# raulmur/ORB_SLAM

Measured on AMD Instinct MI355X. Metric: frames/s ORB extract+match @640x480, 1000 kp, higher is better.
Workload: dtype u8; 1 GPU; vga: 640x480 grayscale stream, 8 levels, nFeatures 1000, S-blocks frames, extract + Hamming top-2 match vs previous frame (BASELINE.json configs[1] + the frame-to-frame match of the metric); resident_frames_per_gpu=2048, lanes=4, parity_checked_frames=0, parity_mismatches=0, library_build_id=8ff709f66bece802, lane_placement=2

## Files before the change

### orb_slam_amd/csrc/k_describe_od.hip

```cpp
#include <algorithm>
#include <type_traits>

#include "orbx_device.h"

namespace orbx {

constexpr int OD_KPW = 4;
constexpr int OD_PITCH = 48, OD_ROWS = 43;
constexpr int OD_WIN_BYTES = OD_PITCH * OD_ROWS;
constexpr int OD_CHUNKS = OD_ROWS * 3;
constexpr int OD_WAVES = DESC_WAVES;
constexpr int OD_TAIL = 512;

typedef int v4i __attribute__((ext_vector_type(4)));
typedef float f2v __attribute__((ext_vector_type(2)));
__device__ __forceinline__ int float_bits(float v) { return __builtin_bit_cast(int, v); }
__host__ __device__ constexpr int od_col0(int ct) { return ct == 0 ? 0 : ct == 1 ? 16 : 24; }
__host__ __device__ constexpr int od_row0(int rt) { return rt == 0 ? 0 : rt == 1 ? 16 : 21; }
typedef const void __attribute__((address_space(1))) * gptr_t;
typedef void __attribute__((address_space(3))) * lptr_t;

constexpr int od_tap(int t) { return t >= 0 && t <= 6 ? (int)((0x12223137312212ull >> (8 * t)) & 255ull) : 0; }
constexpr uint32_t od_taps4(int t0) { return (uint32_t)od_tap(t0) | (uint32_t)od_tap(t0 + 1) << 8 | (uint32_t)od_tap(t0 + 2) << 16 | (uint32_t)od_tap(t0 + 3) << 24; }
struct OdTables {
    uint32_t mask[256];
    float pat[256][4];
    uint32_t trow[3][64][4];
    uint32_t tcol[3][64][4];
};
constexpr uint32_t c_pattern_host[256] = {
#include "orb_pattern_packed.inc"
};
constexpr OdTables make_od_tables() {
    OdTables T{};
    for (int t = 0; t < 256; t++) {
        const int r = t >> 3, c = t & 7;
        const int v = r - HALF_PATCH, av = v < 0 ? -v : v;
        const int um = r < 31 ? (int)((UMAX_NIBBLES >> (4 * (av & 15))) & 15ull) : -1;
        uint32_t mask = 0;
        for (int kk = 0; kk < 4; kk++) {
            const int u = 4 * c + kk - HALF_PATCH;
            if ((u < 0 ? -u : u) <= um) mask |= 0xFFu << (8 * kk);
        }
        T.mask[t] = mask;
        const uint32_t pk = c_pattern_host[t];
        for (int e = 0; e < 4; e++) T.pat[t][e] = (float)(int)(int8_t)(uint8_t)(pk >> (8 * e));
    }
    for (int c = 0; c < 3; c++)
        for (int l = 0; l < 64; l++)
            for (int v = 0; v < 4; v++) {
                const int n = l & 15, g = l >> 4;
                T.trow[c][l][v] = od_taps4(16 * g + 4 * v - (od_col0(c) + n) - 1);
                T.tcol[c][l][v] = od_taps4(16 * v + 4 * g - (od_row0(c) + n));
            }
    return T;
}
static __device__ __constant__ OdTables c_od = make_od_tables();

template <bool FMA, bool GATHER>
__device__ __forceinline__ void k_describe_od_body(const Batch& b) {
    __shared__ __attribute__((aligned(16))) float s_pat[256 * 4];
    __shared__ __attribute__((aligned(16))) uint32_t s_mask[256];
    __shared__ __attribute__((aligned(16))) uint8_t s_win[OD_WAVES * OD_KPW * OD_WIN_BYTES + OD_TAIL];
    const DevGeom& g = b.g;
    int frame, wgi;
    if (!frame_item(b, blockIdx.x, (g.nquads + OD_WAVES - 1) / OD_WAVES, frame, wgi)) return;
    const int tid = threadIdx.x, lane = tid & 63;
    const int grp = lane >> 4, li = lane & 15;
    const float4 pat_first = *reinterpret_cast<const float4*>(c_od.pat[tid & 255]);
    const uint32_t mask_first = c_od.mask[tid & 255];
    const int32_t* counts = b.level_count + frame * MAX_LEVELS;
    const int quad = wgi * OD_WAVES + wave_id();
    const bool live = quad < g.nquads;
    const int level = __builtin_amdgcn_readfirstlane(find_level(g.quad_bases, live ? quad : 0));
    const LevelGeom& LG = g.lv[level];
    struct { int w, h, stride, plane_off, sel_base, quad_base, wvec; float scale, kp_size; } L = {
        __builtin_amdgcn_readfirstlane(LG.w), __builtin_amdgcn_readfirstlane(LG.h), __builtin_amdgcn_readfirstlane(LG.stride),
        __builtin_amdgcn_readfirstlane(LG.plane_off), __builtin_amdgcn_readfirstlane(LG.sel_base), __builtin_amdgcn_readfirstlane(LG.quad_base),
        __builtin_amdgcn_readfirstlane(LG.blur_wvec),
        __builtin_bit_cast(float, __builtin_amdgcn_readfirstlane(__builtin_bit_cast(int, LG.scale))),
        __builtin_bit_cast(float, __builtin_amdgcn_readfirstlane(__builtin_bit_cast(int, LG.kp_size)))};
    const int k0 = (quad - L.quad_base) * OD_KPW;
    Cand kp;
    typedef int v8i_s __attribute__((ext_vector_type(8)));
    v8i_s s_cnt0, s_cnt1;
    int st0;
    {
        const int sel_cap = __builtin_amdgcn_readfirstlane(LG.sel_cap);
        const int ks = __builtin_amdgcn_readfirstlane(max(min(k0, sel_cap - OD_KPW), 0));
        const Cand* kp4 = b.sel + ((long long)frame * g.frame_sel + L.sel_base + ks);
        const int32_t* stp = b.status + frame;
        static_assert(MAX_LEVELS >= 16, "the per-level counts are fetched as two s_load_dwordx8");
        v8i_s kq;
        int sst;
        asm volatile("s_load_dwordx8 %0, %4, 0x0\n\ts_load_dwordx8 %1, %5, 0x0\n\ts_load_dwordx8 %2, %5, 0x20\n\ts_load_dword %3, %6, 0x0\n\ts_waitcnt lgkmcnt(0)"
                     : "=&s"(kq), "=&s"(s_cnt0), "=&s"(s_cnt1), "=&s"(sst) : "s"(kp4), "s"(counts), "s"(stp) : "memory");
        st0 = sst;
        const int e = min(max(k0 + grp, 0), sel_cap - 1) - ks;
        kp.pos = (uint32_t)(e == 0 ? kq[0] : e == 1 ? kq[2] : e == 2 ? kq[4] : kq[6]);
        kp.resp = __builtin_bit_cast(float, e == 0 ? kq[1] : e == 1 ? kq[3] : e == 2 ? kq[5] : kq[7]);
    }
    static_assert(OD_WAVES * 64 == 256, "one table entry per thread");
    reinterpret_cast<float4*>(s_pat)[tid] = pat_first;
    s_mask[tid] = mask_first;
    int out_base = 0, total = 0, cnt = 0;
    for (int l = 0; l < g.nlevels; l++) {
        int c = 0;
#pragma unroll
        for (int i = 0; i < 8; i++) { if (l == i) c = s_cnt0[i]; if (l == 8 + i) c = s_cnt1[i]; }
        if (l < level) out_base += c;
        if (l == level) cnt = c;
        total += c;
    }
    const bool work = live && k0 < cnt && total <= b.cap && __builtin_amdgcn_readfirstlane(st0) == ORBX_OK;
    const bool valid = work && k0 + grp < cnt;
    const int k = valid ? k0 + grp : (work ? k0 : 0);
    if (!valid) {
        kp.pos = (uint32_t)__builtin_amdgcn_readlane((int)kp.pos, 0);
        kp.resp = __builtin_bit_cast(float, __builtin_amdgcn_readlane(__builtin_bit_cast(int, kp.resp), 0));
    }
    if (quad == 0 && lane == 0) {
        int st = st0, tot = total;
        if (tot > b.cap) { st = ORBX_ERR_CAPACITY; tot = 0; }
        b.out_n[frame] = st == ORBX_OK ? tot : 0;
        if (b.out_status) b.out_status[frame] = st;
    }
    if (!work) return;
    const int x = kp.pos & 0xFFFF, y = kp.pos >> 16;
    const uint8_t* plain;
    unsigned pstride;
    int wlim;
    if (level == 0) {
        if constexpr (GATHER) {
            long long s0;
            plain = level0_src(b, frame, s0);
            pstride = (unsigned)s0;
        } else { pstride = (unsigned)b.img_row_stride; plain = b.img + (long long)frame * b.img_frame_stride; }
        wlim = (int)min((long long)pstride, (long long)((L.w + 15) & ~15));
    } else { pstride = (unsigned)L.stride; plain = b.pyr + (long long)frame * g.frame_plane_bytes + L.plane_off; wlim = L.stride; }
    uint8_t* const win0 = s_win + wave_id() * OD_KPW * OD_WIN_BYTES;

    int erow[3], ecol[3];
    unsigned eoff[3];
#pragma unroll
    for (int n = 0; n < 3; n++) {
        const int e = 64 * n + lane;
        erow[n] = (e * 171) >> 9;
        ecol[n] = 16 * (e - 3 * erow[n]);
        eoff[n] = __umul24((unsigned)erow[n], pstride) + (unsigned)ecol[n];
    }
    uint32_t fixmask = 0;
#pragma unroll
    for (int q = 0; q < OD_KPW; q++) {
        if (q > 0 && k0 + q >= cnt) continue;
        const unsigned posq = (unsigned)__builtin_amdgcn_readlane((int)kp.pos, 16 * q);
        const int xq = posq & 0xFFFF, yq = posq >> 16;
        const int xs = (xq - 22) & ~3;
        if (xs < 0 || xs + 48 > wlim || xq + 21 >= L.w) fixmask |= 1u << q;
        if (xq < 18 || xq + 18 >= L.w || yq < 18 || yq + 21 >= L.h) fixmask |= 16u << q;
        if (xs >= 0 && xs + 48 <= wlim && yq >= 21 && yq + 21 < L.h) {
            const uint8_t* srcq = plain + (__umul24((unsigned)(yq - 21), pstride) + (unsigned)xs);
#pragma unroll
            for (int n = 0; n < 3; n++)
                if (n < 2 || lane < OD_CHUNKS - 128)
                    __builtin_amdgcn_global_load_lds((gptr_t)(srcq + eoff[n]), (lptr_t)(win0 + q * OD_WIN_BYTES + 1024 * n), 16, 0, 0);
            continue;
        }
#pragma unroll
        for (int n = 0; n < 3; n++) {
            if (n == 2 && lane >= OD_CHUNKS - 128) continue;
            int Y = yq - 21 + erow[n];
            Y = Y < 0 ? -Y : Y;
            Y = Y >= L.h ? 2 * L.h - 2 - Y : Y;
            Y = min(max(Y, 0), L.h - 1);
            const int X = min(max(xs + ecol[n], 0), wlim - 16);
            __builtin_amdgcn_global_load_lds((gptr_t)(plain + (__umul24((unsigned)Y, pstride) + (unsigned)X)), (lptr_t)(win0 + q * OD_WIN_BYTES + 1024 * n), 16, 0, 0);
        }
    }
    fixmask = (uint32_t)__builtin_amdgcn_readfirstlane((int)fixmask);
    asm volatile("s_waitcnt lgkmcnt(0)\n\ts_barrier" ::: "memory");

    const int n16 = li, g4 = grp;
    v4i Trow[3], Tcol[3];
#pragma unroll
    for (int c = 0; c < 3; c++) {
        Trow[c] = *reinterpret_cast<const v4i*>(c_od.trow[c][lane]);
        Tcol[c] = *reinterpret_cast<const v4i*>(c_od.tcol[c][lane]);
    }
    asm volatile("s_waitcnt vmcnt(0)" ::: "memory");
    wave_lds_fence();

    if (fixmask & 15u) {
#pragma unroll 1
        for (int q = 0; q < OD_KPW; q++) {
            if (!((fixmask >> q) & 1u)) continue;
            const unsigned posq = (unsigned)__builtin_amdgcn_readlane((int)kp.pos, 16 * q);
            const int xq = posq & 0xFFFF;
            const int xs = (xq - 22) & ~3;
            uint8_t* W = win0 + q * OD_WIN_BYTES;
#pragma unroll 1
            for (int j = 0; j < 3; j += 2) {
                const int X0 = xs + 16 * j, Xc = min(max(X0, 0), wlim - 16);
                if (X0 >= 0 && X0 + 16 <= wlim && X0 + 15 < L.w) continue;
                uint32_t nv[3];
#pragma unroll
                for (int it = 0; it < 3; it++) {
                    const int item = 64 * it + lane;
                    const int r = item >> 2, d = item & 3;
                    uint32_t v = 0;
                    if (item < 4 * OD_ROWS) {
#pragma unroll
                        for (int bb = 0; bb < 4; bb++) {
                            const int X = X0 + 4 * d + bb;
                            int Xr = X < 0 ? -X : (X >= L.w ? 2 * L.w - 2 - X : X);
                            Xr = min(max(Xr, 0), L.w - 1);
                            const int src = (Xr >= Xc && Xr < Xc + 16) ? 16 * j + (Xr - Xc) : min(max(Xr - xs, 0), OD_PITCH - 1);
                            v |= (uint32_t)W[r * OD_PITCH + src] << (8 * bb);
                        }
                    }
                    nv[it] = v;
                }
                wave_lds_fence();
#pragma unroll
                for (int it = 0; it < 3; it++) {
                    const int item = 64 * it + lane;
                    if (item < 4 * OD_ROWS) *reinterpret_cast<uint32_t*>(W + (item >> 2) * OD_PITCH + 16 * j + 4 * (item & 3)) = nv[it];
                }
                wave_lds_fence();
            }
        }
    }

    const int xs_own = (x - 22) & ~3, cx = x - xs_own;
    const uint8_t* Wown = win0 + grp * OD_WIN_BYTES;
    int m10, m01;
    {
        const int rsub = li >> 1, hf = li & 1;
        const int boff = cx - HALF_PATCH + 16 * hf;
        const int sh = boff & 3;
        const uint32_t* rowp = reinterpret_cast<const uint32_t*>(Wown + (6 + rsub) * OD_PITCH + (boff & ~3));
        uint32_t uw[4];
#pragma unroll
        for (int d = 0; d < 4; d++) uw[d] = (uint32_t)(16 * hf + 4 * d) * 0x01010101u + 0x03020100u;
        uint32_t a_su = 0, a_si = 0, a_r = 0;
#pragma unroll
        for (int n = 0; n < 4; n++) {
            const uint32_t* p = rowp + (8 * n) * (OD_PITCH / 4);
            uint32_t dw[5];
#pragma unroll
            for (int d = 0; d < 5; d++) dw[d] = p[d];
            const uint4 mk = *reinterpret_cast<const uint4*>(s_mask + (8 * (8 * n + rsub) + 4 * hf));
            const uint32_t mm[4] = {mk.x, mk.y, mk.z, mk.w};
            uint32_t srow = 0;
#pragma unroll
            for (int d = 0; d < 4; d++) {
                const uint32_t Im = __builtin_amdgcn_alignbyte(dw[d + 1], dw[d], (uint32_t)sh) & mm[d];
                srow = __builtin_amdgcn_udot4(Im, 0x01010101u, srow, false);
                a_su = __builtin_amdgcn_udot4(Im, uw[d], a_su, false);
            }
            a_si += srow;
            a_r = __umul24(srow, (uint32_t)(8 * n)) + a_r;
        }
        const int p10 = (int)a_su - HALF_PATCH * (int)a_si;
        const int p01 = (rsub - HALF_PATCH) * (int)a_si + (int)a_r;
        m10 = row16_sum(p10); m01 = row16_sum(p01);
    }
    const float angle = fast_atan2_deg((float)m01, (float)m10);
    wave_lds_fence();

    const unsigned a_off = (unsigned)(n16 * OD_PITCH + 16 * g4);
    const unsigned o_off = (unsigned)((n16 + 3) * OD_PITCH + 4 + 4 * g4);
    auto blur_window = [&](auto EDGE, uint8_t* W, int xs, int yq) {
        constexpr bool edge = decltype(EDGE)::value;
        v4i A[3];
        {
            const unsigned ra = (unsigned)(uintptr_t)(lptr_t)(W + a_off);
            asm volatile("ds_read_b128 %0, %3\n\tds_read_b128 %1, %3 offset:768\n\tds_read_b128 %2, %3 offset:1536\n\ts_waitcnt lgkmcnt(0)"
                         : "=&v"(A[0]), "=&v"(A[1]), "=&v"(A[2]) : "v"(ra) : "memory");
        }
#pragma unroll
        for (int t = 0; t < 3; t++) {
            A[t].x = (int)((uint32_t)A[t].x ^ 0x80808080u); A[t].y = (int)((uint32_t)A[t].y ^ 0x80808080u);
            A[t].z = (int)((uint32_t)A[t].z ^ 0x80808080u); A[t].w = (int)((uint32_t)A[t].w ^ 0x80808080u);
        }
#pragma unroll
        for (int ct = 0; ct < 3; ct++) {
            const v4i c128 = {128, 128, 128, 128};
            v4i z[3];
#pragma unroll
            for (int t = 0; t < 3; t++) z[t] = __builtin_amdgcn_mfma_i32_16x16x64_i8(A[t], Trow[ct], c128, 0, 0, 0);
            int h4[4] = {0, 0, 0, 0}, l4[4] = {0, 0, 0, 0};
#pragma unroll
            for (int t = 0; t < 3; t++) {
                const uint32_t p01 = __builtin_amdgcn_perm((uint32_t)z[t][1], (uint32_t)z[t][0], 0x05010400u);
                const uint32_t p23 = __builtin_amdgcn_perm((uint32_t)z[t][3], (uint32_t)z[t][2], 0x05010400u);
                l4[t] = (int)(__builtin_amdgcn_perm(p23, p01, 0x05040100u) ^ 0x80808080u);
                h4[t] = (int)__builtin_amdgcn_perm(p23, p01, 0x07060302u);
            }
            const v4i HI = {h4[0], h4[1], h4[2], h4[3]}, LO = {l4[0], l4[1], l4[2], l4[3]};
            const int X0 = xs + 4 + od_col0(ct) + 4 * g4;
            const uint32_t tw = X0 < L.wvec ? 1u : 0u;
            const uint32_t cadd = (uint32_t)(257 * 32896 + 0x7FFF) + (tw ^ 1u);
            uint32_t keepc = 0;
            if (edge) {
#pragma unroll
                for (int bb = 0; bb < 4; bb++) keepc |= ((unsigned)(X0 + bb) < (unsigned)L.w ? 0u : 0xFFu) << (8 * bb);
            }
#pragma unroll
            for (int rt = 0; rt < 3; rt++) {
                const v4i zero = {0, 0, 0, 0};
                v4i acc = __builtin_amdgcn_mfma_i32_16x16x64_i8(HI, Tcol[rt], zero, 0, 0, 0);
#pragma unroll
                for (int i = 0; i < 4; i++) acc[i] = (int)(((uint32_t)acc[i] << 8) + cadd);
                acc = __builtin_amdgcn_mfma_i32_16x16x64_i8(LO, Tcol[rt], acc, 0, 0, 0);
                uint32_t qv[4];
#pragma unroll
                for (int i = 0; i < 4; i++) {
                    const uint32_t t = (uint32_t)acc[i];
                    qv[i] = t + ((t >> 16) & tw);
                }
                const us2v lo2 = __builtin_elementwise_min(as_us2v(__builtin_amdgcn_perm(qv[1], qv[0], 0x07060302u)), as_us2v(0x00FF00FFu));
                const us2v hi2 = __builtin_elementwise_min(as_us2v(__builtin_amdgcn_perm(qv[3], qv[2], 0x07060302u)), as_us2v(0x00FF00FFu));
                uint32_t o = __builtin_amdgcn_perm(__builtin_bit_cast(uint32_t, hi2), __builtin_bit_cast(uint32_t, lo2), 0x06040200u);
                uint32_t* dst = reinterpret_cast<uint32_t*>(W + o_off + (od_row0(rt) * OD_PITCH + od_col0(ct)));
                if (edge) {
                    const int Y = yq - 18 + od_row0(rt) + n16;
                    const uint32_t keep = (unsigned)Y < (unsigned)L.h ? keepc : 0xFFFFFFFFu;
                    o = (o & ~keep) | (*dst & keep);
                }
                *dst = o;
            }
        }
    };
#pragma unroll 1
    for (int q = 0; q < OD_KPW; q++) {
        if (q > 0 && k0 + q >= cnt) continue;
        const unsigned posq = (unsigned)__builtin_amdgcn_readlane((int)kp.pos, 16 * q);
        const int xq = posq & 0xFFFF, yq = posq >> 16;
        const int xs = (xq - 22) & ~3;
        uint8_t* W = win0 + q * OD_WIN_BYTES;
        if ((fixmask >> (4 + q)) & 1u) blur_window(std::true_type{}, W, xs, yq);
        else blur_window(std::false_type{}, W, xs, yq);
    }
    wave_lds_fence();

    const float factorPI = (float)(3.14159265358979323846 / 180.f);
    float sn, cs;
    sincosf_orb(angle * factorPI, &sn, &cs);
    const float4* pat = reinterpret_cast<const float4*>(s_pat) + li;
    uint32_t mybits = 0;
    {
        const uint8_t* ctr = Wown + 21 * OD_PITCH + cx;
        const f2v SC = {sn, cs};
        auto rotate = [&](f2v pt) -> f2v {
            f2v m1, r;
            asm("v_pk_mul_f32 %0, %1, %2 op_sel:[1,1] op_sel_hi:[1,0]" : "=v"(m1) : "v"(pt), "v"(SC));
            if (FMA) asm("v_pk_fma_f32 %0, %1, %2, %3 op_sel:[0,0,0] op_sel_hi:[0,1,1] neg_hi:[0,0,1]" : "=v"(r) : "v"(pt), "v"(SC), "v"(m1));
            else {
                f2v m0;
                asm("v_pk_mul_f32 %0, %1, %2 op_sel:[0,0] op_sel_hi:[0,1]" : "=v"(m0) : "v"(pt), "v"(SC));
                asm("v_pk_add_f32 %0, %1, %2 neg_hi:[0,1]" : "=v"(r) : "v"(m0), "v"(m1));
            }
            return r;
        };
        f2v MAGIC = {12582912.0f, 12582912.0f};
        asm("" : "+v"(MAGIC));
        const uint32_t ctr_a = (uint32_t)(uintptr_t)(lptr_t)ctr - (uint32_t)(OD_PITCH * 0x400000 + 0x4B400000);
        typedef const uint8_t __attribute__((address_space(3))) * lbyte_t;
#pragma unroll
        for (int j = 15; j >= 0; j--) {
            const float4 P = pat[16 * j];
            f2v r0 = rotate((f2v){P.x, P.y}), r1 = rotate((f2v){P.z, P.w});
            r0 = r0 + MAGIC;
            r1 = r1 + MAGIC;
            const float r0y = r0.x, r0x = r0.y, r1y = r1.x, r1x = r1.y;
            const uint32_t o0 = (uint32_t)(__mul24(float_bits(r0y), OD_PITCH) + float_bits(r0x));
            const uint32_t o1 = (uint32_t)(__mul24(float_bits(r1y), OD_PITCH) + float_bits(r1x));
            const uint32_t v0 = *(lbyte_t)(uintptr_t)(ctr_a + o0), v1 = *(lbyte_t)(uintptr_t)(ctr_a + o1);
            asm("v_cmp_lt_u32_e32 vcc, %1, %2\n\tv_addc_co_u32_e32 %0, vcc, %0, %0, vcc" : "+v"(mybits) : "v"(v0), "v"(v1) : "vcc");
        }
    }
    uint32_t half = mybits;
    auto stage = [&](auto S) {
        constexpr int s = decltype(S)::value;
        constexpr uint32_t M0 = s == 8 ? 0x00FFu : s == 4 ? 0x0F0Fu : s == 2 ? 0x3333u : 0x5555u;
        const bool hi = (li & s) != 0;
        const uint32_t yv = (uint32_t)__builtin_amdgcn_ds_swizzle((int)half, (s << 10) | 0x1F);
        const uint32_t ysh = hi ? (yv >> s) : (yv << s);
        const uint32_t mk = hi ? (~M0 & 0xFFFFu) : M0;
        half = (half & mk) | (ysh & ~mk & 0xFFFFu);
    };
    stage(std::integral_constant<int, 8>{}); stage(std::integral_constant<int, 4>{});
    stage(std::integral_constant<int, 2>{}); stage(std::integral_constant<int, 1>{});
    if (!valid) return;
    const int out_idx = out_base + k;
    reinterpret_cast<uint16_t*>(b.out_desc + ((long long)frame * b.cap + out_idx) * 32)[li] = (uint16_t)half;
    if (li == 0) {
        orbx_keypoint o;
        o.x = (float)x; o.y = (float)y;
        if (level != 0) { o.x = o.x * L.scale; o.y = o.y * L.scale; }
        o.size = L.kp_size;
        o.angle = angle;
        o.response = kp.resp;
        o.octave = level;
        o.class_id = -1;
        b.out_kps[(long long)frame * b.cap + out_idx] = o;
    }
}
template <bool FMA>
__global__ __launch_bounds__(OD_WAVES * 64) void k_describe_od(Batch b) { k_describe_od_body<FMA, false>(b); }
template <bool FMA>
__global__ __launch_bounds__(OD_WAVES * 64) void k_describe_od_gather(Batch b) { k_describe_od_body<FMA, true>(b); }

bool describe_od_supported(const Batch& b, const HostGeom& hg) {
    const DevGeom& g = hg.g;
    for (int l = 0; l < g.nlevels; l++)
        if (g.lv[l].w < 64 || g.lv[l].h < 44) return false;
    const long long wlim0 = std::min<long long>(level0_min_stride(b), (g.lv[0].w + 15) & ~15);
    return wlim0 >= 64 && wlim0 >= g.lv[0].w;
}

int launch_describe_od(const Batch& b, const HostGeom& hg, hipStream_t stream) {
    const DevGeom& g = hg.g;
    const dim3 grid(frame_item_blocks(b, (g.nquads + OD_WAVES - 1) / OD_WAVES)), block(OD_WAVES * 64);
    if (g.fp_contract) hipLaunchKernelGGL(b.img_tab ? k_describe_od_gather<true> : k_describe_od<true>, grid, block, 0, stream, b);
    else hipLaunchKernelGGL(b.img_tab ? k_describe_od_gather<false> : k_describe_od<false>, grid, block, 0, stream, b);
    return hipGetLastError() == hipSuccess ? ORBX_OK : ORBX_ERR_DEVICE;
}

}
```

Measured before the change: 431,400 frames/s.

## Pair keypoint windows in MFMA blur to pack partial edge tiles together

Restructures the separable Gaussian blur of the four descriptor windows per wave so that windows are processed in pairs. The third, partially used column and row tiles of two windows, and a shared corner tile for all four, are packed into a single MFMA, using new zero-padded tap tables. This is meant to cut the wasted MFMA work on overlapping 16-wide edge tiles. It also switches byte packing to SDWA v_min_u16 and adds a waves_per_eu(4) occupancy hint. The price is more complex index bookkeeping, edge-case handling when paired windows disagree on bounds, and added register pressure.

```diff
diff --git a/orb_slam_amd/csrc/k_describe_od.hip b/orb_slam_amd/csrc/k_describe_od.hip
--- a/orb_slam_amd/csrc/k_describe_od.hip
+++ b/orb_slam_amd/csrc/k_describe_od.hip
@@ -15,8 +15,6 @@
 typedef int v4i __attribute__((ext_vector_type(4)));
 typedef float f2v __attribute__((ext_vector_type(2)));
 __device__ __forceinline__ int float_bits(float v) { return __builtin_bit_cast(int, v); }
-__host__ __device__ constexpr int od_col0(int ct) { return ct == 0 ? 0 : ct == 1 ? 16 : 24; }
-__host__ __device__ constexpr int od_row0(int rt) { return rt == 0 ? 0 : rt == 1 ? 16 : 21; }
 typedef const void __attribute__((address_space(1))) * gptr_t;
 typedef void __attribute__((address_space(3))) * lptr_t;
 
@@ -50,8 +48,13 @@
         for (int l = 0; l < 64; l++)
             for (int v = 0; v < 4; v++) {
                 const int n = l & 15, g = l >> 4;
-                T.trow[c][l][v] = od_taps4(16 * g + 4 * v - (od_col0(c) + n) - 1);
-                T.tcol[c][l][v] = od_taps4(16 * v + 4 * g - (od_row0(c) + n));
+                if (c < 2) {
+                    T.trow[c][l][v] = od_taps4(16 * g + 4 * v - (16 * c + n) - 1);
+                    T.tcol[c][l][v] = od_taps4(16 * v + 4 * g - (16 * c + n));
+                } else {
+                    T.trow[c][l][v] = g == 2 && n < 8 ? od_taps4(4 * v - n - 1) : g == 3 && n >= 8 ? od_taps4(4 * v - (n - 8) - 1) : 0u;
+                    T.tcol[c][l][v] = v == 2 && n < 5 ? od_taps4(4 * g - n) : v == 3 && n >= 8 && n < 13 ? od_taps4(4 * g - (n - 8)) : 0u;
+                }
             }
     return T;
 }
@@ -269,78 +272,128 @@
     wave_lds_fence();
 
     const unsigned a_off = (unsigned)(n16 * OD_PITCH + 16 * g4);
-    const unsigned o_off = (unsigned)((n16 + 3) * OD_PITCH + 4 + 4 * g4);
-    auto blur_window = [&](auto EDGE, uint8_t* W, int xs, int yq) {
-        constexpr bool edge = decltype(EDGE)::value;
-        v4i A[3];
+    const unsigned a_offp = g4 == 3 ? (unsigned)(OD_WIN_BYTES + n16 * OD_PITCH + 32) : a_off;
+    const unsigned o_own = (unsigned)((n16 + 3) * OD_PITCH + 4 + 4 * g4);
+    const unsigned o_prow = (unsigned)((n16 >= 8 ? OD_WIN_BYTES : 0) + ((n16 & 7) + 35) * OD_PITCH + 4 + 4 * g4);
+    const unsigned o_pcol = (unsigned)((g4 >= 2 ? OD_WIN_BYTES : 0) + (n16 + 3) * OD_PITCH + 36 + 4 * (g4 & 1));
+    const unsigned o_corner = (unsigned)((n16 < 8 ? 2 : 0) * OD_WIN_BYTES + (g4 >= 2 ? OD_WIN_BYTES : 0) + ((n16 & 7) + 35) * OD_PITCH + 36 + 4 * (g4 & 1));
+    int xsw[OD_KPW], yqw[OD_KPW];
+    uint32_t tww[OD_KPW];
+    bool genw[OD_KPW];
+#pragma unroll
+    for (int q = 0; q < OD_KPW; q++) {
+        const unsigned posq = (unsigned)__builtin_amdgcn_readlane((int)kp.pos, 16 * q);
+        xsw[q] = ((int)(posq & 0xFFFF) - 22) & ~3;
+        yqw[q] = (int)(posq >> 16);
+        const bool lo = xsw[q] + 4 < L.wvec, hi = xsw[q] + 40 < L.wvec;
+        const bool liveq = q == 0 || k0 + q < cnt;
+        tww[q] = liveq ? (lo ? 1u : 0u) : tww[q > 0 ? q - 1 : 0];
+        genw[q] = liveq && (((fixmask >> (4 + q)) & 1u) || lo != hi);
+    }
+    constexpr uint32_t CADD = 257 * 32896 + 0x7FFF;
+    const v4i c128 = {128, 128, 128, 128}, zero = {0, 0, 0, 0};
+    auto row_pass = [&](const v4i (&A)[3], const v4i& T, v4i& HI, v4i& LO) {
+        v4i z[3];
+#pragma unroll
+        for (int t = 0; t < 3; t++) z[t] = __builtin_amdgcn_mfma_i32_16x16x64_i8(A[t], T, c128, 0, 0, 0);
+#pragma unroll
+        for (int t = 0; t < 3; t++) {
+            const uint32_t p01 = __builtin_amdgcn_perm((uint32_t)z[t][1], (uint32_t)z[t][0], 0x05010400u);
+            const uint32_t p23 = __builtin_amdgcn_perm((uint32_t)z[t][3], (uint32_t)z[t][2], 0x05010400u);
+            LO[t] = (int)(__builtin_amdgcn_perm(p23, p01, 0x05040100u) ^ 0x80808080u);
+            HI[t] = (int)__builtin_amdgcn_perm(p23, p01, 0x07060302u);
+        }
+    };
+    const uint32_t c255 = 255;
+    auto epilogue = [&](auto GEN, const v4i& HI, const v4i& LO, const v4i& T, uint8_t* dst, int xs_l, int yq_l, int cb, int ro, uint32_t twu) {
+        constexpr bool gen = decltype(GEN)::value;
+        uint32_t tw = twu, keep = 0;
+        if (gen) {
+            const int X0 = xs_l + 4 + cb;
+            tw = X0 < L.wvec ? 1u : 0u;
+            uint32_t keepc = 0;
+#pragma unroll
+            for (int bb = 0; bb < 4; bb++) keepc |= ((unsigned)(X0 + bb) < (unsigned)L.w ? 0u : 0xFFu) << (8 * bb);
+            keep = (unsigned)(yq_l - 18 + ro) < (unsigned)L.h ? keepc : 0xFFFFFFFFu;
+        }
+        const uint32_t cadd = CADD + (tw ^ 1u);
+        v4i acc = __builtin_amdgcn_mfma_i32_16x16x64_i8(HI, T, zero, 0, 0, 0);
+#pragma unroll
+        for (int i = 0; i < 4; i++) acc[i] = (int)(((uint32_t)acc[i] << 8) + cadd);
+        acc = __builtin_amdgcn_mfma_i32_16x16x64_i8(LO, T, acc, 0, 0, 0);
+        uint32_t q[4];
+#pragma unroll
+        for (int i = 0; i < 4; i++) {
+            const uint32_t t = (uint32_t)acc[i];
+            q[i] = t + ((t >> 16) & tw);
+        }
+        uint32_t o;
+        asm("v_min_u16_sdwa %0, %1, %2 dst_sel:BYTE_0 dst_unused:UNUSED_PAD src0_sel:WORD_1 src1_sel:DWORD" : "=v"(o) : "v"(q[0]), "v"(c255));
+        asm("v_min_u16_sdwa %0, %1, %2 dst_sel:BYTE_1 dst_unused:UNUSED_PRESERVE src0_sel:WORD_1 src1_sel:DWORD" : "+v"(o) : "v"(q[1]), "v"(c255));
+        asm("v_min_u16_sdwa %0, %1, %2 dst_sel:BYTE_2 dst_unused:UNUSED_PRESERVE src0_sel:WORD_1 src1_sel:DWORD" : "+v"(o) : "v"(q[2]), "v"(c255));
+        asm("v_min_u16_sdwa %0, %1, %2 dst_sel:BYTE_3 dst_unused:UNUSED_PRESERVE src0_sel:WORD_1 src1_sel:DWORD" : "+v"(o) : "v"(q[3]), "v"(c255));
+        uint32_t* d = reinterpret_cast<uint32_t*>(dst);
+        if (gen) o = (o & ~keep) | (*d & keep);
+        *d = o;
+    };
+    int hc[2] = {0, 0}, lc[2] = {0, 0};
+    auto blur_pair = [&](auto GEN, int p, int xs0, int yq0, int xs1, int yq1, uint32_t twu) {
+        uint8_t* W = win0 + 2 * p * OD_WIN_BYTES;
+        v4i A0[3], A1[3];
         {
-            const unsigned ra = (unsigned)(uintptr_t)(lptr_t)(W + a_off);
-            asm volatile("ds_read_b128 %0, %3\n\tds_read_b128 %1, %3 offset:768\n\tds_read_b128 %2, %3 offset:1536\n\ts_waitcnt lgkmcnt(0)"
-                         : "=&v"(A[0]), "=&v"(A[1]), "=&v"(A[2]) : "v"(ra) : "memory");
-        }
-#pragma unroll
-        for (int t = 0; t < 3; t++) {
-            A[t].x = (int)((uint32_t)A[t].x ^ 0x80808080u); A[t].y = (int)((uint32_t)A[t].y ^ 0x80808080u);
-            A[t].z = (int)((uint32_t)A[t].z ^ 0x80808080u); A[t].w = (int)((uint32_t)A[t].w ^ 0x80808080u);
-        }
-#pragma unroll
-        for (int ct = 0; ct < 3; ct++) {
-            const v4i c128 = {128, 128, 128, 128};
-            v4i z[3];
-#pragma unroll
-            for (int t = 0; t < 3; t++) z[t] = __builtin_amdgcn_mfma_i32_16x16x64_i8(A[t], Trow[ct], c128, 0, 0, 0);
-            int h4[4] = {0, 0, 0, 0}, l4[4] = {0, 0, 0, 0};
-#pragma unroll
-            for (int t = 0; t < 3; t++) {
-                const uint32_t p01 = __builtin_amdgcn_perm((uint32_t)z[t][1], (uint32_t)z[t][0], 0x05010400u);
-                const uint32_t p23 = __builtin_amdgcn_perm((uint32_t)z[t][3], (uint32_t)z[t][2], 0x05010400u);
-                l4[t] = (int)(__builtin_amdgcn_perm(p23, p01, 0x05040100u) ^ 0x80808080u);
-                h4[t] = (int)__builtin_amdgcn_perm(p23, p01, 0x07060302u);
+            const unsigned r0 = (unsigned)(uintptr_t)(lptr_t)(W + a_offp), r1 = (unsigned)(uintptr_t)(lptr_t)(W + OD_WIN_BYTES + a_off);
+            asm volatile("ds_read_b128 %0, %6\n\tds_read_b128 %1, %6 offset:768\n\tds_read_b128 %2, %6 offset:1536\n\t"
+                         "ds_read_b128 %3, %7\n\tds_read_b128 %4, %7 offset:768\n\tds_read_b128 %5, %7 offset:1536\n\ts_waitcnt lgkmcnt(0)"
+                         : "=&v"(A0[0]), "=&v"(A0[1]), "=&v"(A0[2]), "=&v"(A1[0]), "=&v"(A1[1]), "=&v"(A1[2]) : "v"(r0), "v"(r1) : "memory");
+        }
+#pragma unroll
+        for (int t = 0; t < 3; t++)
+#pragma unroll
+            for (int e = 0; e < 4; e++) { A0[t][e] = (int)((uint32_t)A0[t][e] ^ 0x80808080u); A1[t][e] = (int)((uint32_t)A1[t][e] ^ 0x80808080u); }
+        const int xs_r = n16 >= 8 ? xs1 : xs0, yq_r = n16 >= 8 ? yq1 : yq0;
+        const int xs_c = g4 >= 2 ? xs1 : xs0, yq_c = g4 >= 2 ? yq1 : yq0;
+        {
+            v4i HP, LP;
+            row_pass(A0, Trow[2], HP, LP);
+            HP[3] = HP[2]; LP[3] = LP[2];
+#pragma unroll
+            for (int rt = 0; rt < 2; rt++)
+                epilogue(GEN, HP, LP, Tcol[rt], W + o_pcol + 16 * rt * OD_PITCH, xs_c, yq_c, 32 + 4 * (g4 & 1), 16 * rt + n16, twu);
+            if (p == 0) { hc[0] = HP[2]; lc[0] = LP[2]; hc[1] = HP[2]; lc[1] = LP[2]; }
+            else { hc[1] = HP[2]; lc[1] = LP[2]; }
+        }
+#pragma unroll
+        for (int ct = 0; ct < 2; ct++) {
+            v4i H0, L0, H1, L1;
+            row_pass(A0, Trow[ct], H0, L0);
+            row_pass(A1, Trow[ct], H1, L1);
+            H0[3] = H1[2]; L0[3] = L1[2];
+            H1[3] = H1[2]; L1[3] = L1[2];
+#pragma unroll
+            for (int rt = 0; rt < 2; rt++) {
+                epilogue(GEN, H0, L0, Tcol[rt], W + o_own + (16 * rt * OD_PITCH + 16 * ct), xs0, yq0, 16 * ct + 4 * g4, 16 * rt + n16, twu);
+                epilogue(GEN, H1, L1, Tcol[rt], W + OD_WIN_BYTES + o_own + (16 * rt * OD_PITCH + 16 * ct), xs1, yq1, 16 * ct + 4 * g4, 16 * rt + n16, twu);
             }
-            const v4i HI = {h4[0], h4[1], h4[2], h4[3]}, LO = {l4[0], l4[1], l4[2], l4[3]};
-            const int X0 = xs + 4 + od_col0(ct) + 4 * g4;
-            const uint32_t tw = X0 < L.wvec ? 1u : 0u;
-            const uint32_t cadd = (uint32_t)(257 * 32896 + 0x7FFF) + (tw ^ 1u);
-            uint32_t keepc = 0;
-            if (edge) {
-#pragma unroll
-                for (int bb = 0; bb < 4; bb++) keepc |= ((unsigned)(X0 + bb) < (unsigned)L.w ? 0u : 0xFFu) << (8 * bb);
-            }
-#pragma unroll
-            for (int rt = 0; rt < 3; rt++) {
-                const v4i zero = {0, 0, 0, 0};
-                v4i acc = __builtin_amdgcn_mfma_i32_16x16x64_i8(HI, Tcol[rt], zero, 0, 0, 0);
-#pragma unroll
-                for (int i = 0; i < 4; i++) acc[i] = (int)(((uint32_t)acc[i] << 8) + cadd);
-                acc = __builtin_amdgcn_mfma_i32_16x16x64_i8(LO, Tcol[rt], acc, 0, 0, 0);
-                uint32_t qv[4];
-#pragma unroll
-                for (int i = 0; i < 4; i++) {
-                    const uint32_t t = (uint32_t)acc[i];
-                    qv[i] = t + ((t >> 16) & tw);
-                }
-                const us2v lo2 = __builtin_elementwise_min(as_us2v(__builtin_amdgcn_perm(qv[1], qv[0], 0x07060302u)), as_us2v(0x00FF00FFu));
-                const us2v hi2 = __builtin_elementwise_min(as_us2v(__builtin_amdgcn_perm(qv[3], qv[2], 0x07060302u)), as_us2v(0x00FF00FFu));
-                uint32_t o = __builtin_amdgcn_perm(__builtin_bit_cast(uint32_t, hi2), __builtin_bit_cast(uint32_t, lo2), 0x06040200u);
-                uint32_t* dst = reinterpret_cast<uint32_t*>(W + o_off + (od_row0(rt) * OD_PITCH + od_col0(ct)));
-                if (edge) {
-                    const int Y = yq - 18 + od_row0(rt) + n16;
-                    const uint32_t keep = (unsigned)Y < (unsigned)L.h ? keepc : 0xFFFFFFFFu;
-                    o = (o & ~keep) | (*dst & keep);
-                }
-                *dst = o;
-            }
+            epilogue(GEN, H0, L0, Tcol[2], W + o_prow + 16 * ct, xs_r, yq_r, 16 * ct + 4 * g4, 32 + (n16 & 7), twu);
         }
     };
+    const int nlive = min(cnt - k0, OD_KPW);
 #pragma unroll 1
-    for (int q = 0; q < OD_KPW; q++) {
-        if (q > 0 && k0 + q >= cnt) continue;
-        const unsigned posq = (unsigned)__builtin_amdgcn_readlane((int)kp.pos, 16 * q);
-        const int xq = posq & 0xFFFF, yq = posq >> 16;
-        const int xs = (xq - 22) & ~3;
-        uint8_t* W = win0 + q * OD_WIN_BYTES;
-        if ((fixmask >> (4 + q)) & 1u) blur_window(std::true_type{}, W, xs, yq);
-        else blur_window(std::false_type{}, W, xs, yq);
+    for (int p = 0; p < 2; p++) {
+        if (p > 0 && nlive <= 2) continue;
+        const int xs0 = p ? xsw[2] : xsw[0], yq0 = p ? yqw[2] : yqw[0], xs1 = p ? xsw[3] : xsw[1], yq1 = p ? yqw[3] : yqw[1];
+        const uint32_t tw0 = p ? tww[2] : tww[0], tw1 = p ? tww[3] : tww[1];
+        if ((p ? genw[2] || genw[3] : genw[0] || genw[1]) || tw0 != tw1) blur_pair(std::true_type{}, p, xs0, yq0, xs1, yq1, tw0);
+        else blur_pair(std::false_type{}, p, xs0, yq0, xs1, yq1, tw0);
+    }
+    {
+        const bool gen = genw[0] || genw[1] || genw[2] || genw[3] || tww[0] != tww[1] || tww[0] != tww[2] || tww[0] != tww[3];
+        const int wsc = (n16 < 8 ? 2 : 0) + (g4 >= 2 ? 1 : 0);
+        const int xs_k = wsc == 0 ? xsw[0] : wsc == 1 ? xsw[1] : wsc == 2 ? xsw[2] : xsw[3];
+        const int yq_k = wsc == 0 ? yqw[0] : wsc == 1 ? yqw[1] : wsc == 2 ? yqw[2] : yqw[3];
+        const v4i HC = {hc[1], hc[1], hc[1], hc[0]}, LC = {lc[1], lc[1], lc[1], lc[0]};
+        if (gen) epilogue(std::true_type{}, HC, LC, Tcol[2], win0 + o_corner, xs_k, yq_k, 32 + 4 * (g4 & 1), 32 + (n16 & 7), tww[0]);
+        else epilogue(std::false_type{}, HC, LC, Tcol[2], win0 + o_corner, xs_k, yq_k, 32 + 4 * (g4 & 1), 32 + (n16 & 7), tww[0]);
     }
     wave_lds_fence();
 
@@ -408,9 +461,9 @@
     }
 }
 template <bool FMA>
-__global__ __launch_bounds__(OD_WAVES * 64) void k_describe_od(Batch b) { k_describe_od_body<FMA, false>(b); }
+__global__ __launch_bounds__(OD_WAVES * 64) __attribute__((amdgpu_waves_per_eu(4))) void k_describe_od(Batch b) { k_describe_od_body<FMA, false>(b); }
 template <bool FMA>
-__global__ __launch_bounds__(OD_WAVES * 64) void k_describe_od_gather(Batch b) { k_describe_od_body<FMA, true>(b); }
+__global__ __launch_bounds__(OD_WAVES * 64) __attribute__((amdgpu_waves_per_eu(4))) void k_describe_od_gather(Batch b) { k_describe_od_body<FMA, true>(b); }
 
 bool describe_od_supported(const Batch& b, const HostGeom& hg) {
     const DevGeom& g = hg.g;
```

Measured after the change: 451,000 frames/s (median of 6 runs). 1.05x the previous value.
